# menyifang/MIMO

Hardware: NVIDIA H100
Metric: frames/sec @ 512x512x24f, 20 DDIM steps (higher is better)
Workload: dtype fp16

## Files before the change

### include/mimo_b200.h

```cpp
#ifndef MIMO_B200_H_
#define MIMO_B200_H_

#include <stdint.h>

#ifdef __cplusplus
extern "C" {
#endif

#define MIMO_OK 0
#define MIMO_ERR_ARG (-1)
#define MIMO_ERR_CUDA (-2)
#define MIMO_ERR_DEVICE (-3)

#define MIMO_F16 0
#define MIMO_BF16 1

#define MIMO_ACT_NONE 0
#define MIMO_ACT_SILU 1
#define MIMO_ACT_GEGLU 2

const char* mimo_version(void);
const char* mimo_last_error(void);
int mimo_device_check(int dev);
int mimo_abi_sizeof(int which);

typedef struct {
  const void* bias;
  const void* rowvec;
  int64_t rows_per_group;
  int64_t ld_rowvec;
  const void* residual;
  int64_t ld_res;
  float scale;
  int act;
} mimo_epilogue;

typedef struct {
  const void* a;
  int64_t lda;
  const void* a1;
  int64_t lda1;
  const void* w;
  int64_t ldw;
  void* out;
  int64_t ldo;
  int32_t M, N, K;
  int32_t K1;
  int32_t dtype;
  mimo_epilogue ep;
  void* workspace;
  int64_t workspace_bytes;
} mimo_gemm_params;
int mimo_gemm(const mimo_gemm_params* p, void* stream);
int mimo_gemm_geglu_granule(int32_t N);

typedef struct {
  const void* a;
  int64_t lda;
  const float* a_scale;
  const void* w;
  int64_t ldw;
  const float* w_scale;
  void* out;
  int64_t ldo;
  int32_t M, N, K;
  int32_t dtype;
  mimo_epilogue ep;
  void* workspace;
  int64_t workspace_bytes;
} mimo_gemm_e4m3_params;
int mimo_gemm_e4m3(const mimo_gemm_e4m3_params* p, void* stream);

typedef struct {
  const void* x0;
  int32_t c0;
  const void* x1;
  int32_t c1;
  const void* w;
  void* out;
  int64_t ldo;
  int32_t n, h, w_, cout;
  int32_t dtype;
  mimo_epilogue ep;
  void* workspace;
  int64_t workspace_bytes;
} mimo_conv3x3_params;
int mimo_conv3x3(const mimo_conv3x3_params* p, void* stream);
// ... 155 lines not shown
```

### mimo_b200/csrc/gemm_wgmma.cu

```cuda
#include <cuda_runtime.h>

#include <cudaTypedefs.h>

#include "../../include/mimo_b200.h"
#include "host_util.h"
#include "ptx.cuh"
#include "wgmma.cuh"

namespace mimo {

constexpr int BM = 128;
constexpr int BK = 64;
constexpr int kGemmThreads = 320;
constexpr int kChunk = 8192;

struct EpiArgs {
  const void* bias;
  const void* rowvec;
  long long rows_per_group;
  long long ld_rowvec;
  float scale;
  int act;
  float* partial;
};
// ... 23 lines not shown
  static constexpr int kResBytes = kResSlots * kChunk;
  static constexpr int kBarBytes = 512;
  static constexpr int kFixed = kBarBytes + 2048  + (kE4m3 ? 3072  : 0) + kOutBytes + kResBytes;
  static constexpr int kMaxStages = (BN >= 256) ? 4 : (BN >= 160 ? 5 : (BN >= 128 ? 6 : 8));
  static constexpr int kFit = (227 * 1024 - kFixed) / kStageBytes;
  static constexpr int kStages = kFit < kMaxStages ? kFit : kMaxStages;
  static constexpr int kSmemBytes = kStages * kStageBytes + kFixed;
  static_assert(kStages >= 3, "pipeline too shallow");
};

template <int BN, bool kBf16, bool kRes>
__global__ void __launch_bounds__(kGemmThreads, 1)
gemm_wgmma_kernel(const __grid_constant__ CUtensorMap tmA0, const __grid_constant__ CUtensorMap tmA1,
                  const __grid_constant__ CUtensorMap tmB, const __grid_constant__ CUtensorMap tmOut,
                  const __grid_constant__ CUtensorMap tmRes, int M, int N, int num_m_tiles, int num_n_tiles,
                  int num_k_blocks, ConvGeom g, EpiArgs ep) {
  constexpr bool kE4m3 = false;
  constexpr const float* a_scale = nullptr;
  constexpr const float* w_scale = nullptr;
#include "gemm_wgmma_body.cuh"
}

template <int BN, bool kBf16, bool kRes>
__global__ void __launch_bounds__(kGemmThreads, 1)
gemm_e4m3_kernel(const __grid_constant__ CUtensorMap tmA0, const __grid_constant__ CUtensorMap tmA1,
                 const __grid_constant__ CUtensorMap tmB, const __grid_constant__ CUtensorMap tmOut,
                 const __grid_constant__ CUtensorMap tmRes, int M, int N, int num_m_tiles, int num_n_tiles,
                 int num_k_blocks, ConvGeom g, EpiArgs ep, const float* __restrict__ a_scale,
                 const float* __restrict__ w_scale) {
  constexpr bool kE4m3 = true;
#include "gemm_wgmma_body.cuh"
}


template <bool kBf16>
__global__ void __launch_bounds__(256)
splitk_reduce_kernel(const float* __restrict__ part, int splits, long long M, int N, const void* __restrict__ bias,
                     const void* __restrict__ rowvec, long long rpg, long long ld_rowvec,
                     const void* __restrict__ res, long long ld_res, float scale, int act, void* __restrict__ out,
                     long long ldo) {
  using C = Cvt<kBf16>;
  using T = typename C::T;
  pdl_launch_dependents();
  pdl_wait();
  const int nv = N >> 3;
  const long long idx = blockIdx.x * static_cast<long long>(blockDim.x) + threadIdx.x;
  if (idx >= M * nv) return;
  const long long row = idx / nv;
  const int col = static_cast<int>(idx - row * nv) * 8;
  float a[8] = {0.f, 0.f, 0.f, 0.f, 0.f, 0.f, 0.f, 0.f};
  for (int s = 0; s < splits; ++s) {
    const float4* p = reinterpret_cast<const float4*>(part + (static_cast<long long>(s) * M + row) * N + col);
    const float4 u0 = p[0], u1 = p[1];
    a[0] += u0.x, a[1] += u0.y, a[2] += u0.z, a[3] += u0.w;
    a[4] += u1.x, a[5] += u1.y, a[6] += u1.z, a[7] += u1.w;
  }
  float cst[8] = {0.f, 0.f, 0.f, 0.f, 0.f, 0.f, 0.f, 0.f};
  auto add_vec = [&](const T* v, float* dst, bool scaled_fma) {
    const uint4 b = *reinterpret_cast<const uint4*>(v);
    const uint32_t w[4] = {b.x, b.y, b.z, b.w};
#pragma unroll
    for (int j = 0; j < 4; ++j) {
      const float2 t = C::unpack(w[j]);
      if (scaled_fma) {
        dst[2 * j] = fmaf(t.x, scale, dst[2 * j]);
        dst[2 * j + 1] = fmaf(t.y, scale, dst[2 * j + 1]);
// ... 47 lines not shown
  }
  const int tiles = mt * nt;
  const int grid = tiles < num_sms() ? tiles : num_sms();
  cudaError_t e = launch_k(kern, dim3(grid), dim3(kGemmThreads), Cfg::kSmemBytes, st, m.a0, m.a1, m.b, m.out, m.res, M, N, mt,
                           nt, nkb, g, ep);
  if (e == cudaSuccess) e = cudaGetLastError();
  if (e != cudaSuccess) return set_cuda_error("gemm launch", e);
  return MIMO_OK;
}

template <bool kBf16>
static int launch_bn(int bn, bool res, const Maps& m, int M, int N, int mt, int nt, int nkb, const ConvGeom& g,
                     const EpiArgs& ep, cudaStream_t st) {
  switch (bn) {
    case 64:
      return res ? launch_cfg<64, kBf16, true>(m, M, N, mt, nt, nkb, g, ep, st)
                 : launch_cfg<64, kBf16, false>(m, M, N, mt, nt, nkb, g, ep, st);
    case 128:
      return res ? launch_cfg<128, kBf16, true>(m, M, N, mt, nt, nkb, g, ep, st)
                 : launch_cfg<128, kBf16, false>(m, M, N, mt, nt, nkb, g, ep, st);
    case 160:
      return res ? launch_cfg<160, kBf16, true>(m, M, N, mt, nt, nkb, g, ep, st)
                 : launch_cfg<160, kBf16, false>(m, M, N, mt, nt, nkb, g, ep, st);
    case 192:
      return res ? launch_cfg<192, kBf16, true>(m, M, N, mt, nt, nkb, g, ep, st)
                 : launch_cfg<192, kBf16, false>(m, M, N, mt, nt, nkb, g, ep, st);
    case 256:
      return res ? launch_cfg<256, kBf16, true>(m, M, N, mt, nt, nkb, g, ep, st)
                 : launch_cfg<256, kBf16, false>(m, M, N, mt, nt, nkb, g, ep, st);
  }
  return set_error(MIMO_ERR_ARG, "gemm: unsupported BN");
}

int pick_bn(int N, bool geglu, long long m_tiles);

template <bool kBf16>
static int launch_e4m3(int bn, bool res, const Maps& m, int M, int N, int mt, int nt, int nkb, const ConvGeom& g,
                       const EpiArgs& ep, const float* a_scale, const float* w_scale, cudaStream_t st) {
  auto run = [&](auto kern, int smem) -> int {
    static bool attr_done[2][2][2] = {};
    bool& done = attr_done[bn == 256][kBf16][res];
    if (!done) {
      cudaError_t e = cudaFuncSetAttribute(kern, cudaFuncAttributeMaxDynamicSharedMemorySize, smem);
      if (e != cudaSuccess) return set_cuda_error("cudaFuncSetAttribute(gemm_e4m3)", e);
      done = true;
    }
    const int tiles = mt * nt;
    const int grid = tiles < num_sms() ? tiles : num_sms();
    cudaError_t e = launch_k(kern, dim3(grid), dim3(kGemmThreads), smem, st, m.a0, m.a1, m.b, m.out, m.res, M, N, mt, nt,
                             nkb, g, ep, a_scale, w_scale);
    if (e == cudaSuccess) e = cudaGetLastError();
    if (e != cudaSuccess) return set_cuda_error("gemm_e4m3 launch", e);
    return MIMO_OK;
  };
  if (bn == 192)
    return res ? run(gemm_e4m3_kernel<192, kBf16, true>, GemmCfg<192, true, true>::kSmemBytes)
               : run(gemm_e4m3_kernel<192, kBf16, false>, GemmCfg<192, false, true>::kSmemBytes);
  if (bn == 256)
    return res ? run(gemm_e4m3_kernel<256, kBf16, true>, GemmCfg<256, true, true>::kSmemBytes)
               : run(gemm_e4m3_kernel<256, kBf16, false>, GemmCfg<256, false, true>::kSmemBytes);
  return set_error(MIMO_ERR_ARG, "mimo_gemm_e4m3: unsupported BN");
}

static int pick_bn_e4m3(int N, bool geglu) {
  if (geglu) return pick_bn(N, true, 1 << 20);
  const int pad256 = (N + 255) / 256 * 256 - N, pad192 = (N + 191) / 192 * 192 - N;
  return pad192 < pad256 ? 192 : 256;
}

static int g_force_bn = 0;

int pick_bn(int N, bool geglu, long long m_tiles) {
  if (g_force_bn) return g_force_bn;
  if (geglu) {
    if (N % 256 == 0) return 256;
    if (N % 128 == 0) return 128;
    return 64;
  }
  const int cands[5] = {256, 192, 160, 128, 64};
  int best = 64;
  double best_eff = -1.0;
  for (int i = 0; i < 5; ++i) {
    const int bn = cands[i];
    const int nt = (N + bn - 1) / bn;
    double eff = static_cast<double>(N) / (static_cast<double>(nt) * bn);
    const long long tiles = m_tiles * nt;
    if (tiles < num_sms() && bn > 64) eff *= 0.5 + 0.5 * static_cast<double>(tiles) / num_sms();
    if (eff > best_eff + 1e-9) {
      best_eff = eff;
      best = bn;
    }
  }
  return best;
}

static EpiArgs make_epi(const mimo_epilogue& e, int N) {
  EpiArgs a;
  a.bias = e.bias;
  a.rowvec = e.rowvec;
  a.rows_per_group = e.rows_per_group > 0 ? e.rows_per_group : 1;
  if (a.rows_per_group > 0x7fffffffLL) a.rows_per_group = 0x7fffffffLL;
  a.ld_rowvec = e.ld_rowvec > 0 ? e.ld_rowvec : N;
  a.scale = e.scale;
  a.act = e.act;
  a.partial = nullptr;
  return a;
}

static int g_splitk = 0;

static int launch_reduce(int dtype, const float* part, int splits, long long M, int N, const mimo_epilogue& e, void* out,
                         long long ldo, cudaStream_t st) {
  const long long total = M * (N / 8);
  const unsigned blocks = div_up(total, 256);
  const long long rpg = e.rows_per_group > 0 ? e.rows_per_group : 1;
  const long long ldr = e.ld_rowvec > 0 ? e.ld_rowvec : N;
  cudaError_t err = dtype == MIMO_BF16
                        ? launch_k(splitk_reduce_kernel<true>, dim3(blocks), dim3(256), 0, st, part, splits, M, N, e.bias,
                                   e.rowvec, rpg, ldr, e.residual, static_cast<long long>(e.ld_res), e.scale, e.act, out, ldo)
                        : launch_k(splitk_reduce_kernel<false>, dim3(blocks), dim3(256), 0, st, part, splits, M, N, e.bias,
                                   e.rowvec, rpg, ldr, e.residual, static_cast<long long>(e.ld_res), e.scale, e.act, out, ldo);
  if (err == cudaSuccess) err = cudaGetLastError();
  if (err != cudaSuccess) return set_cuda_error("split-K reduce launch", err);
  return MIMO_OK;
}

}

using namespace mimo;

extern "C" int mimo_debug_splitk(int mode) {
  g_splitk = mode;
  return 0;
}

extern "C" int mimo_debug_force_bn(int bn) {
  g_force_bn = bn;
  return 0;
}

extern "C" int mimo_gemm_geglu_granule(int32_t N) { return pick_bn(N, true, 1 << 20) / 2; }

extern "C" int mimo_gemm(const mimo_gemm_params* p, void* stream) {
  if (!p || !p->a || !p->w || !p->out) return set_error(MIMO_ERR_ARG, "mimo_gemm: null pointer");
  if (p->M <= 0 || p->N <= 0 || p->K <= 0) return set_error(MIMO_ERR_ARG, "mimo_gemm: empty problem");
  if ((p->K % 8) || (p->lda % 8) || (p->ldw % 8) || (p->N % 8) || (p->ldo % 8))
    return set_error(MIMO_ERR_ARG, "mimo_gemm: K, N, lda, ldw, ldo must be multiples of 8");
  if (p->ep.residual && (p->ep.ld_res % 8)) return set_error(MIMO_ERR_ARG, "mimo_gemm: ld_res % 8 != 0");
  const bool geglu = p->ep.act == MIMO_ACT_GEGLU;
  if (geglu && (p->ep.residual || p->ep.rowvec))
    return set_error(MIMO_ERR_ARG, "mimo_gemm: GEGLU takes neither a residual nor a row vector");
  if (int rc = ensure_device()) return rc;
  const int mt = (p->M + BM - 1) / BM;
  const int K1 = p->a1 ? p->K1 : 0;
  if (K1 < 0 || (K1 % 8) || (p->a1 && (p->lda1 % 8))) return set_error(MIMO_ERR_ARG, "mimo_gemm: K1/lda1 % 8 != 0");
  const int kb0 = (p->K + BK - 1) / BK;
  const int kb1 = (K1 + BK - 1) / BK;
  const int nkb = kb0 + kb1;
  int bn = pick_bn(p->N, geglu, mt);
  int splits = 1;
  if (!geglu && g_splitk && p->workspace && !g_force_bn) {
    const int bn_wide = pick_bn(p->N, false, 1 << 20);
    splits = pick_splits(static_cast<long long>(mt) * ((p->N + bn_wide - 1) / bn_wide), nkb, p->M, p->N, p->workspace_bytes);
    if (splits > 1) bn = bn_wide;
  }
  if (geglu && (p->N % bn)) return set_error(MIMO_ERR_ARG, "mimo_gemm: GEGLU needs N % tile == 0");
  const int nt = (p->N + bn - 1) / bn;
  const bool res = p->ep.residual != nullptr && !geglu && splits == 1;

  Maps m;
  const uint64_t adim[2] = {static_cast<uint64_t>(p->K), static_cast<uint64_t>(p->M)};
  const uint64_t astr[1] = {static_cast<uint64_t>(p->lda) * 2};
  const uint32_t abox[2] = {BK, BM};
  if (int rc = encode_tmap(&m.a0, p->dtype, 2, p->a, adim, astr, abox)) return rc;
  m.a1 = m.a0;
  if (K1) {
    const uint64_t a1dim[2] = {static_cast<uint64_t>(K1), static_cast<uint64_t>(p->M)};
    const uint64_t a1str[1] = {static_cast<uint64_t>(p->lda1) * 2};
    if (int rc = encode_tmap(&m.a1, p->dtype, 2, p->a1, a1dim, a1str, abox)) return rc;
  }
  const uint64_t bdim[2] = {static_cast<uint64_t>(p->K + K1), static_cast<uint64_t>(p->N)};
  const uint64_t bstr[1] = {static_cast<uint64_t>(p->ldw) * 2};
  const uint32_t bbox[2] = {BK, static_cast<uint32_t>(bn)};
  if (int rc = encode_tmap(&m.b, p->dtype, 2, p->w, bdim, bstr, bbox)) return rc;
  const int n_out = geglu ? p->N / 2 : p->N;
  const uint64_t odim[2] = {static_cast<uint64_t>(n_out), static_cast<uint64_t>(p->M)};
  const uint64_t ostr[1] = {static_cast<uint64_t>(p->ldo) * 2};
  const uint32_t obox[2] = {32, BM};
  if (int rc = encode_tmap(&m.out, p->dtype, 2, p->out, odim, ostr, obox, 64)) return rc;
  m.res = m.out;
  if (res) {
    const uint64_t rstr[1] = {static_cast<uint64_t>(p->ep.ld_res) * 2};
    if (int rc = encode_tmap(&m.res, p->dtype, 2, p->ep.residual, odim, rstr, obox, 64)) return rc;
  }

  ConvGeom g = {};
  g.kb0 = kb0;
  g.kb1 = kb1;
  g.c0 = p->K;
  g.chunk_bytes = kChunk;
  g.splits = splits;
  g.kb_split = (nkb + splits - 1) / splits;
  EpiArgs ep = make_epi(p->ep, p->N);
  cudaStream_t st = static_cast<cudaStream_t>(stream);
  if (splits > 1) {
    ep.bias = ep.rowvec = nullptr;
    ep.act = MIMO_ACT_NONE;
    ep.scale = 1.0f;
    ep.partial = static_cast<float*>(p->workspace);
  }
  const int rc = p->dtype == MIMO_BF16 ? launch_bn<true>(bn, res, m, p->M, p->N, mt, nt, nkb, g, ep, st)
                                       : launch_bn<false>(bn, res, m, p->M, p->N, mt, nt, nkb, g, ep, st);
  if (rc || splits == 1) return rc;
  return launch_reduce(p->dtype, ep.partial, splits, p->M, p->N, p->ep, p->out, p->ldo, st);
}

extern "C" int mimo_gemm_e4m3(const mimo_gemm_e4m3_params* p, void* stream) {
  if (!p || !p->a || !p->w || !p->out || !p->a_scale || !p->w_scale)
    return set_error(MIMO_ERR_ARG, "mimo_gemm_e4m3: null pointer");
  if (p->M <= 0 || p->N <= 0 || p->K <= 0) return set_error(MIMO_ERR_ARG, "mimo_gemm_e4m3: empty problem");
  if ((p->K % 16) || (p->lda % 16) || (p->ldw % 16))
    return set_error(MIMO_ERR_ARG, "mimo_gemm_e4m3: K, lda, ldw must be multiples of 16");
  if ((p->N % 8) || (p->ldo % 8)) return set_error(MIMO_ERR_ARG, "mimo_gemm_e4m3: N, ldo must be multiples of 8");
  if ((reinterpret_cast<uintptr_t>(p->a) | reinterpret_cast<uintptr_t>(p->w) | reinterpret_cast<uintptr_t>(p->out) |
       reinterpret_cast<uintptr_t>(p->ep.residual)) % 16)
    return set_error(MIMO_ERR_ARG, "mimo_gemm_e4m3: a, w, out, residual must be 16-byte aligned");
  if (p->ep.residual && (p->ep.ld_res % 8)) return set_error(MIMO_ERR_ARG, "mimo_gemm_e4m3: ld_res % 8 != 0");
  if (p->workspace || p->workspace_bytes) return set_error(MIMO_ERR_ARG, "mimo_gemm_e4m3: split-K is not supported");
  const bool geglu = p->ep.act == MIMO_ACT_GEGLU;
  if (geglu && (p->ep.residual || p->ep.rowvec))
    return set_error(MIMO_ERR_ARG, "mimo_gemm_e4m3: GEGLU takes neither a residual nor a row vector");
  const int bn = pick_bn_e4m3(p->N, geglu);
  if (geglu && (p->N % bn)) return set_error(MIMO_ERR_ARG, "mimo_gemm_e4m3: GEGLU needs N % tile == 0");
  if (bn != 192 && bn != 256) return set_error(MIMO_ERR_ARG, "mimo_gemm_e4m3: GEGLU needs N % 256 == 0");
  if (int rc = ensure_device()) return rc;
  const int mt = (p->M + BM - 1) / BM;
  const int nt = (p->N + bn - 1) / bn;
  const int nkb = (p->K + 2 * BK - 1) / (2 * BK);
  const bool res = p->ep.residual != nullptr && !geglu;

  Maps m;
  const uint64_t adim[2] = {static_cast<uint64_t>(p->K), static_cast<uint64_t>(p->M)};
  const uint64_t astr[1] = {static_cast<uint64_t>(p->lda)};
// ... 40 lines not shown
  if (g.TH < 1) g.TH = 1;
  g.TN = BM / (g.TW * g.TH);
  if (g.TN > p->n) g.TN = p->n;
  if (g.TN < 1) g.TN = 1;
  if (g.TN > 1 && g.TH != p->h) g.TN = 1;
  g.tiles_w = (p->w_ + g.TW - 1) / g.TW;
  g.tiles_h = (p->h + g.TH - 1) / g.TH;
  const int tiles_n = (p->n + g.TN - 1) / g.TN;
  g.ctot = p->c0 + c1;
  g.c0 = p->c0;
  g.kb0 = (p->c0 + BK - 1) / BK;
  g.kb1 = (c1 + BK - 1) / BK;
  g.a_bytes = g.TW * g.TH * g.TN * BK * 2;
  g.chunk_bytes = g.TW * g.TH * g.TN * 64;
  g.ntaps = ntaps;
  for (int t = 0; t < 9; ++t) {
    g.tdx[t] = t < ntaps ? tdx[t] : 0;
    g.tdy[t] = t < ntaps ? tdy[t] : 0;
  }
  const int mt = g.tiles_w * g.tiles_h * tiles_n;
  const int nkb = ntaps * (g.kb0 + g.kb1);
  const long long Mrows = static_cast<long long>(p->n) * p->h * p->w_;
  if (Mrows > 0x7fffffffLL) return set_error(MIMO_ERR_ARG, "mimo_conv: too many pixels");
  int bn = pick_bn(p->cout, false, mt);
  int splits = 1;
  if (g_splitk && p->workspace && !g_force_bn && sx == 1 && sy == 1 && p->ldo == p->cout) {
    const int bn_wide = pick_bn(p->cout, false, 1 << 20);
    splits = pick_splits(static_cast<long long>(mt) * ((p->cout + bn_wide - 1) / bn_wide), nkb, Mrows, p->cout,
                         p->workspace_bytes);
    if (splits > 1) bn = bn_wide;
  }
  g.splits = splits;
  g.kb_split = (nkb + splits - 1) / splits;
  const int nt = (p->cout + bn - 1) / bn;
  const bool res = p->ep.residual != nullptr && splits == 1;

  Maps m;
  auto nhwc_map = [&](CUtensorMap* tm, const void* base, int c, long long pitch, uint32_t box_c, int swz, int px,
                      int py, int iw, int ih) {
    const uint64_t dim[4] = {static_cast<uint64_t>(c), static_cast<uint64_t>(p->w_), static_cast<uint64_t>(p->h),
                             static_cast<uint64_t>(p->n)};
    const uint64_t str[3] = {static_cast<uint64_t>(px) * pitch * 2, static_cast<uint64_t>(py) * iw * pitch * 2,
                             static_cast<uint64_t>(ih) * iw * pitch * 2};
    const uint32_t box[4] = {box_c, static_cast<uint32_t>(g.TW), static_cast<uint32_t>(g.TH),
                             static_cast<uint32_t>(g.TN)};
    return encode_tmap(tm, p->dtype, 4, base, dim, str, box, swz);
  };
  if (int rc = nhwc_map(&m.a0, p->x0, p->c0, p->c0, BK, 128, 1, 1, p->w_, p->h)) return rc;
  m.a1 = m.a0;
  if (c1)
    if (int rc = nhwc_map(&m.a1, p->x1, c1, c1, BK, 128, 1, 1, p->w_, p->h)) return rc;
  {
    const uint64_t dim[2] = {static_cast<uint64_t>(ntaps) * g.ctot, static_cast<uint64_t>(p->cout)};
    const uint64_t str[1] = {static_cast<uint64_t>(ntaps) * g.ctot * 2};
    const uint32_t box[2] = {BK, static_cast<uint32_t>(bn)};
    if (int rc = encode_tmap(&m.b, p->dtype, 2, w, dim, str, box)) return rc;
  }
  if (int rc = nhwc_map(&m.out, out, p->cout, p->ldo, 32, 64, sx, sy, ow, oh)) return rc;
  m.res = m.out;
  if (res)
    if (int rc = nhwc_map(&m.res, p->ep.residual, p->cout, p->ep.ld_res, 32, 64, 1, 1, p->w_, p->h)) return rc;

  EpiArgs ep = make_epi(p->ep, p->cout);
  cudaStream_t st = static_cast<cudaStream_t>(stream);
  if (splits > 1) {
    ep.bias = ep.rowvec = nullptr;
    ep.act = MIMO_ACT_NONE;
    ep.scale = 1.0f;
    ep.partial = static_cast<float*>(p->workspace);
  }
  const int rc = p->dtype == MIMO_BF16
                     ? launch_bn<true>(bn, res, m, static_cast<int>(Mrows), p->cout, mt, nt, nkb, g, ep, st)
                     : launch_bn<false>(bn, res, m, static_cast<int>(Mrows), p->cout, mt, nt, nkb, g, ep, st);
  if (rc || splits == 1) return rc;
  return launch_reduce(p->dtype, ep.partial, splits, Mrows, p->cout, p->ep, out, p->ldo, st);
}

static int conv_check(const mimo_conv3x3_params* p, const char* who) {
  if (!p || !p->x0 || !p->w || !p->out) return set_error(MIMO_ERR_ARG, "mimo_conv: null pointer");
  if (p->n <= 0 || p->h <= 0 || p->w_ <= 0 || p->cout <= 0 || p->c0 <= 0)
    return set_error(MIMO_ERR_ARG, "mimo_conv: empty problem");
  const int c1 = p->x1 ? p->c1 : 0;
  if ((p->c0 % 8) || (c1 % 8) || (p->cout % 8) || (p->ldo % 8))
    return set_error(MIMO_ERR_ARG, "mimo_conv: channel counts must be multiples of 8");
  if (p->ep.act == MIMO_ACT_GEGLU) return set_error(MIMO_ERR_ARG, "mimo_conv: GEGLU not supported");
  if (p->ep.residual && (p->ep.ld_res % 8)) return set_error(MIMO_ERR_ARG, "mimo_conv: ld_res % 8 != 0");
  (void)who;
  return ensure_device();
}

extern "C" int mimo_conv3x3(const mimo_conv3x3_params* p, void* stream) {
  if (int rc = conv_check(p, "mimo_conv3x3")) return rc;
  static const signed char dx[9] = {-1, 0, 1, -1, 0, 1, -1, 0, 1};
  static const signed char dy[9] = {-1, -1, -1, 0, 0, 0, 1, 1, 1};
  return conv_launch(p, p->w, 9, dx, dy, p->out, 1, 1, p->w_, p->h, stream);
}

extern "C" int mimo_conv_up2x(const mimo_conv3x3_params* p, void* stream) {
  if (int rc = conv_check(p, "mimo_conv_up2x")) return rc;
  if (p->ep.residual || p->ep.rowvec) return set_error(MIMO_ERR_ARG, "mimo_conv_up2x: bias / activation epilogue only");
  const int ctot = p->c0 + (p->x1 ? p->c1 : 0);
  const size_t esz = 2;
  for (int a = 0; a < 2; ++a)
// ... 12 lines not shown
```

### mimo_b200/csrc/ptx.cuh

```cuda
#pragma once
#include <cuda_fp16.h>
#include <cuda_bf16.h>
#include <cuda.h>
#include <stdint.h>
#include <stdio.h>

namespace mimo {

__device__ __forceinline__ uint32_t smem_u32(const void* p) {
  return static_cast<uint32_t>(__cvta_generic_to_shared(p));
}
__device__ __forceinline__ uint32_t lane_id() { return threadIdx.x & 31u; }

__device__ __forceinline__ bool elect_one() {
  uint32_t pred = 0;
  asm volatile(
      "{\n\t.reg .pred P;\n\telect.sync _|P, 0xffffffff;\n\tselp.u32 %0, 1, 0, P;\n\t}\n"
      : "=r"(pred));
  return pred != 0;
}

__device__ __forceinline__ void pdl_launch_dependents() { asm volatile("griddepcontrol.launch_dependents;" ::: "memory"); }
__device__ __forceinline__ void pdl_wait() { asm volatile("griddepcontrol.wait;" ::: "memory"); }

// ... 10 lines not shown
}
__device__ __forceinline__ void mbar_arrive(uint64_t* bar) {
  asm volatile("mbarrier.arrive.shared::cta.b64 _, [%0];" ::"r"(smem_u32(bar)) : "memory");
}
__device__ __forceinline__ bool mbar_try_wait(uint64_t* bar, uint32_t parity) {
  uint32_t ok;
  asm volatile(
      "{\n\t.reg .pred p;\n\t"
      "mbarrier.try_wait.parity.shared::cta.b64 p, [%1], %2;\n\t"
      "selp.u32 %0, 1, 0, p;\n\t}\n"
      : "=r"(ok)
      : "r"(smem_u32(bar)), "r"(parity)
      : "memory");
  return ok != 0;
}
__device__ __forceinline__ bool mbar_test(uint64_t* bar, uint32_t parity) {
  uint32_t ok;
  asm volatile(
      "{\n\t.reg .pred p;\n\t"
      "mbarrier.test_wait.parity.shared::cta.b64 p, [%1], %2;\n\t"
      "selp.u32 %0, 1, 0, p;\n\t}\n"
      : "=r"(ok)
      : "r"(smem_u32(bar)), "r"(parity)
      : "memory");
  return ok != 0;
}
__device__ __forceinline__ void mbar_wait(uint64_t* bar, uint32_t parity) {
  uint32_t spins = 0;
  while (!mbar_try_wait(bar, parity)) {
    if (++spins > (1u << 26)) __trap();
  }
}

__device__ __forceinline__ void fence_proxy_async_smem() {
  asm volatile("fence.proxy.async.shared::cta;" ::: "memory");
}

__device__ __forceinline__ void tma_prefetch_desc(const CUtensorMap* m) {
  asm volatile("prefetch.tensormap [%0];" ::"l"(reinterpret_cast<uint64_t>(m)) : "memory");
}
__device__ __forceinline__ void tma_load_2d(void* smem_dst, const CUtensorMap* m, uint64_t* bar,
                                            int32_t c0, int32_t c1) {
  asm volatile(
      "cp.async.bulk.tensor.2d.shared::cluster.global.mbarrier::complete_tx::bytes"
      " [%0], [%1, {%3, %4}], [%2];"
      ::"r"(smem_u32(smem_dst)), "l"(reinterpret_cast<uint64_t>(m)), "r"(smem_u32(bar)), "r"(c0),
      "r"(c1)
      : "memory");
}
__device__ __forceinline__ void tma_load_3d(void* smem_dst, const CUtensorMap* m, uint64_t* bar,
                                            int32_t c0, int32_t c1, int32_t c2) {
  asm volatile(
      "cp.async.bulk.tensor.3d.shared::cluster.global.mbarrier::complete_tx::bytes"
      " [%0], [%1, {%3, %4, %5}], [%2];"
      ::"r"(smem_u32(smem_dst)), "l"(reinterpret_cast<uint64_t>(m)), "r"(smem_u32(bar)), "r"(c0),
      "r"(c1), "r"(c2)
      : "memory");
}
__device__ __forceinline__ void tma_load_4d(void* smem_dst, const CUtensorMap* m, uint64_t* bar,
                                            int32_t c0, int32_t c1, int32_t c2, int32_t c3) {
  asm volatile(
      "cp.async.bulk.tensor.4d.shared::cluster.global.mbarrier::complete_tx::bytes"
      " [%0], [%1, {%3, %4, %5, %6}], [%2];"
      ::"r"(smem_u32(smem_dst)), "l"(reinterpret_cast<uint64_t>(m)), "r"(smem_u32(bar)), "r"(c0),
      "r"(c1), "r"(c2), "r"(c3)
      : "memory");
}

__device__ __forceinline__ void tma_store_2d(const CUtensorMap* m, const void* smem_src, int32_t c0, int32_t c1) {
  asm volatile("cp.async.bulk.tensor.2d.global.shared::cta.bulk_group [%0, {%2, %3}], [%1];"
               ::"l"(reinterpret_cast<uint64_t>(m)), "r"(smem_u32(smem_src)), "r"(c0), "r"(c1)
               : "memory");
}
__device__ __forceinline__ void tma_store_4d(const CUtensorMap* m, const void* smem_src, int32_t c0, int32_t c1,
                                             int32_t c2, int32_t c3) {
  asm volatile("cp.async.bulk.tensor.4d.global.shared::cta.bulk_group [%0, {%2, %3, %4, %5}], [%1];"
               ::"l"(reinterpret_cast<uint64_t>(m)), "r"(smem_u32(smem_src)), "r"(c0), "r"(c1), "r"(c2), "r"(c3)
               : "memory");
}
__device__ __forceinline__ void tma_store_commit() { asm volatile("cp.async.bulk.commit_group;" ::: "memory"); }
__device__ __forceinline__ void tma_store_wait_read0() { asm volatile("cp.async.bulk.wait_group.read 0;" ::: "memory"); }
__device__ __forceinline__ void tma_store_wait_all() { asm volatile("cp.async.bulk.wait_group 0;" ::: "memory"); }

__device__ __forceinline__ void wgmma_fence() { asm volatile("wgmma.fence.sync.aligned;" ::: "memory"); }
__device__ __forceinline__ void wgmma_commit() { asm volatile("wgmma.commit_group.sync.aligned;" ::: "memory"); }
template <int N>
__device__ __forceinline__ void wgmma_wait() {
  asm volatile("wgmma.wait_group.sync.aligned %0;" ::"n"(N) : "memory");
}
template <int N>
__device__ __forceinline__ void reg_fence(float (&d)[N]) {
#pragma unroll
  for (int i = 0; i < N; ++i) asm volatile("" : "+f"(d[i])::"memory");
}

__device__ __forceinline__ void bar_sync(int id, int count) {
  asm volatile("bar.sync %0, %1;" ::"r"(id), "r"(count) : "memory");
}
__device__ __forceinline__ void bar_arrive(int id, int count) {
  asm volatile("bar.arrive %0, %1;" ::"r"(id), "r"(count) : "memory");
}

__device__ __forceinline__ uint64_t make_smem_desc_sw128(uint32_t smem_addr, uint32_t lbo_bytes,
                                                         uint32_t sbo_bytes) {
  uint64_t d = 0;
  d |= static_cast<uint64_t>((smem_addr & 0x3FFFFu) >> 4);
  d |= static_cast<uint64_t>((lbo_bytes >> 4) & 0x3FFFu) << 16;
  d |= static_cast<uint64_t>((sbo_bytes >> 4) & 0x3FFFu) << 32;
  d |= static_cast<uint64_t>(1) << 62;
  return d;
}

__device__ __forceinline__ float ex2_ftz(float x) {
  float y;
  asm("ex2.approx.ftz.f32 %0, %1;" : "=f"(y) : "f"(x));
  return y;
}
__device__ __forceinline__ float silu_f(float x) { return __fdividef(x, 1.0f + __expf(-x)); }
__device__ __forceinline__ float gelu_erf_f(float x) {
  return 0.5f * x * (1.0f + erff(x * 0.70710678118654752440f));
}

__device__ __forceinline__ float gelu_erf_fast(float x) {
  const float z = fabsf(x) * 0.70710678118654752440f;
  float t;
  asm("rcp.approx.ftz.f32 %0, %1;" : "=f"(t) : "f"(fmaf(0.3275911f, z, 1.0f)));
  float poly = fmaf(1.061405429f, t, -1.453152027f);
// ... 44 lines not shown
```

### mimo_b200/lib.py

```python
from __future__ import annotations

import ctypes as C
import os
from pathlib import Path

_PKG = Path(__file__).resolve().parent
LIB_PATH = _PKG / "libmimo_b200.so"

F16, BF16 = 0, 1
ACT_NONE, ACT_SILU, ACT_GEGLU = 0, 1, 2


class MimoError(RuntimeError):
    pass


class Epilogue(C.Structure):
    _fields_ = [
        ("bias", C.c_void_p),
        ("rowvec", C.c_void_p),
        ("rows_per_group", C.c_int64),
        ("ld_rowvec", C.c_int64),
        ("residual", C.c_void_p),
        ("ld_res", C.c_int64),
# ... 98 lines not shown

MAX_PEERS = 8


class ExchangeParams(C.Structure):
    _fields_ = [
        ("peer_src", C.c_void_p * MAX_PEERS), ("peer_ready", C.c_void_p * MAX_PEERS),
        ("ctl", C.c_void_p), ("dst", C.c_void_p), ("residual", C.c_void_p),
        ("mode", C.c_int32), ("G", C.c_int32), ("r", C.c_int32),
        ("b", C.c_int32), ("fl", C.c_int32), ("hw", C.c_int32), ("C", C.c_int32),
        ("dtype", C.c_int32), ("max_blocks", C.c_int32), ("timeout_ms", C.c_int32),
    ]


class CfgMultistepParams(C.Structure):
    _fields_ = [
        ("pred_uncond", C.c_void_p), ("pred_cond", C.c_void_p), ("counter", C.c_void_p), ("frame_stride", C.c_int64),
        ("latents", C.c_void_p), ("count", C.c_int64),
        ("hist_out", C.c_void_p), ("h1", C.c_void_p), ("h2", C.c_void_p), ("noise", C.c_void_p),
        ("guidance", C.c_float), ("a", C.c_float), ("b", C.c_float),
        ("c_x", C.c_float), ("c_m", C.c_float), ("c_1", C.c_float), ("c_2", C.c_float), ("c_n", C.c_float),
        ("dtype", C.c_int32),
    ]


_VP, _I32, _I64, _F = C.c_void_p, C.c_int32, C.c_int64, C.c_float
SYMBOLS = {
    "mimo_version": (C.c_char_p, []),
    "mimo_last_error": (C.c_char_p, []),
    "mimo_device_check": (C.c_int, [C.c_int]),
    "mimo_abi_sizeof": (C.c_int, [C.c_int]),
    "mimo_gemm": (C.c_int, [C.POINTER(GemmParams), _VP]),
    "mimo_gemm_geglu_granule": (C.c_int, [_I32]),
    "mimo_gemm_e4m3": (C.c_int, [C.POINTER(GemmE4m3Params), _VP]),
    "mimo_conv3x3": (C.c_int, [C.POINTER(Conv3x3Params), _VP]),
    "mimo_conv_up2x": (C.c_int, [C.POINTER(Conv3x3Params), _VP]),
    "mimo_im2col3x3": (C.c_int, [_VP, _VP, _I32, _I32, _I32, _I32, _I32, _I32, _I32, _I64, _I32, _VP]),
    "mimo_groupnorm": (C.c_int, [C.POINTER(GroupNormParams), _VP]),
    "mimo_groupnorm_workspace_bytes": (C.c_int64, [C.POINTER(GroupNormParams)]),
    "mimo_groupnorm_window": (C.c_int, [C.POINTER(GroupNormWindowParams), _VP]),
    "mimo_groupnorm_window_partials": (C.c_int, [C.POINTER(GroupNormWindowParams), _VP]),
    "mimo_groupnorm_window_apply": (C.c_int, [C.POINTER(GroupNormWindowParams), _VP]),
    "mimo_groupnorm_window_table_bytes": (C.c_int64, [C.POINTER(GroupNormWindowParams)]),
    "mimo_layernorm": (C.c_int, [_VP, _VP, _VP, _VP, _I64, _I32, _F, _VP, _I64, _I32, _I32, _I32, _VP]),
    "mimo_layernorm_e4m3": (C.c_int, [_VP, _VP, _VP, _VP, _VP, _I64, _I32, _F, _VP, _I64, _I32, _I32, _I32, _VP]),
    "mimo_attn_spatial": (C.c_int, [C.POINTER(AttnParams), _VP]),
    "mimo_attn_temporal": (C.c_int, [C.POINTER(AttnTemporalParams), _VP]),
    "mimo_exchange": (C.c_int, [C.POINTER(ExchangeParams), _VP]),
    "mimo_peer_alloc": (C.c_int, [_I64, C.POINTER(C.c_void_p), C.c_char_p]),
    "mimo_peer_open": (C.c_int, [C.c_char_p, C.POINTER(C.c_void_p)]),
    "mimo_peer_close": (C.c_int, [_VP]),
    "mimo_peer_free": (C.c_int, [_VP]),
    "mimo_ncfhw_to_nhwc": (C.c_int, [_VP, _VP, _I32, _I32, _I32, _I32, _I32, _I32, _I32, _I32, _VP]),
    "mimo_nhwc_to_ncfhw": (C.c_int, [_VP, _VP, _I32, _I32, _I32, _I32, _I32, _I32, _I32, _I32, _VP]),
    "mimo_upsample2x": (C.c_int, [_VP, _VP, _I32, _I32, _I32, _I32, _I32, _VP]),
    "mimo_upsample_nearest": (C.c_int, [_VP, _VP, _I32, _I32, _I32, _I32, _I32, _I32, _I32, _VP]),
    "mimo_softmax_rows": (C.c_int, [_VP, _I64, _I32, _I64, _I32, _VP]),
    "mimo_add": (C.c_int, [_VP, _VP, _VP, _I64, _I32, _VP]),
    "mimo_silu": (C.c_int, [_VP, _VP, _I64, _I32, _VP]),
    "mimo_quick_gelu": (C.c_int, [_VP, _VP, _I64, _I32, _VP]),
    "mimo_composite_frame": (C.c_int, [_VP, _VP, _VP, _VP, _VP, _VP, C.c_double, _VP, _I64, _VP]),
    "mimo_cfg_ddim_step": (C.c_int, [_VP, _VP, _VP, _I64, _VP, _I64, _F, _F, _F, _F, _F, _I32, _VP]),
    "mimo_cfg_ddim_step_noise": (C.c_int, [_VP, _VP, _VP, _I64, _VP, _I64, _F, _F, _F, _F, _F, _VP, _F, _I32, _VP]),
    "mimo_interpolate_frames": (C.c_int, [_VP, _VP, _I32, _I64, _I32, _I32, _I32, _VP]),
    "mimo_cfg_multistep": (C.c_int, [C.POINTER(CfgMultistepParams), _VP]),
}
# ... 36 lines not shown
```

Measured before the change: 8.198.

## Add persistent warp-specialized ping-pong WGMMA GEMM/conv kernel with wider N tiles

Adds a persistent ping-pong kernel. A producer warp issues TMA loads and another warp prefetches the residual. Two consumer warpgroups alternate tiles, so one warpgroup's epilogue overlaps the other's main loop, and registers are rebalanced with setmaxnreg. A heuristic routes non-split GEMMs and 3x3 convs to it with BN of 128, 160 or 192, plus a GEGLU granule path. The goal is to hide epilogue and store latency and to raise tensor-core utilisation, at the cost of more complex synchronisation and shallower pipelines for wide tiles.

```diff
diff --git a/include/mimo_b200.h b/include/mimo_b200.h
--- a/include/mimo_b200.h
+++ b/include/mimo_b200.h
@@ -53,6 +53,7 @@
 } mimo_gemm_params;
 int mimo_gemm(const mimo_gemm_params* p, void* stream);
 int mimo_gemm_geglu_granule(int32_t N);
+int mimo_debug_gemm_schedule(int mode);
 
 typedef struct {
   const void* a;
diff --git a/mimo_b200/csrc/gemm_wgmma.cu b/mimo_b200/csrc/gemm_wgmma.cu
--- a/mimo_b200/csrc/gemm_wgmma.cu
+++ b/mimo_b200/csrc/gemm_wgmma.cu
@@ -79,6 +79,390 @@
 #include "gemm_wgmma_body.cuh"
 }
 
+
+constexpr int kPingPongThreads = 384;
+
+template <int BN, bool kRes>
+struct PingPongCfg {
+  static constexpr int kStageBytes = BM * BK * 2 + BN * BK * 2;
+  static constexpr int kNChunk = BN / 32;
+  static constexpr int kOutBytes = 2 * 2 * kChunk;
+  static constexpr int kResSlots = kRes ? 2 : 0;
+  static constexpr int kResBytes = 2 * kResSlots * kChunk;
+  static constexpr int kBarBytes = 512;
+  static constexpr int kFixed = kBarBytes + 2048  + kOutBytes + kResBytes;
+  static constexpr int kMaxStages = BN >= 160 ? 5 : (BN >= 128 ? 6 : 8);
+  static constexpr int kFit = (227 * 1024 - kFixed) / kStageBytes;
+  static constexpr int kStages = kFit < kMaxStages ? kFit : kMaxStages;
+  static constexpr int kSmemBytes = kStages * kStageBytes + kFixed;
+  static_assert(kStages >= 3, "pipeline too shallow");
+  static_assert(BN <= 192, "BN accumulators per thread must fit the 232-register consumers");
+};
+
+template <int BN, bool kBf16, bool kRes>
+__global__ void __launch_bounds__(kPingPongThreads, 1)
+gemm_pingpong_kernel(const __grid_constant__ CUtensorMap tmA0, const __grid_constant__ CUtensorMap tmA1,
+                     const __grid_constant__ CUtensorMap tmB, const __grid_constant__ CUtensorMap tmOut,
+                     const __grid_constant__ CUtensorMap tmRes, int M, int N, int num_m_tiles, int num_n_tiles,
+                     int num_k_blocks, ConvGeom g, EpiArgs ep, int w_granule) {
+  using Cfg = PingPongCfg<BN, kRes>;
+  using C = Cvt<kBf16>;
+  using T = typename C::T;
+  constexpr int NCHUNK = Cfg::kNChunk;
+  extern __shared__ __align__(1024) uint8_t smem[];
+  uint8_t* sOut = smem + Cfg::kStages * Cfg::kStageBytes;
+  uint8_t* sRes = sOut + Cfg::kOutBytes;
+  uint64_t* bars = reinterpret_cast<uint64_t*>(sRes + Cfg::kResBytes);
+  uint64_t* full_bar = bars;
+  uint64_t* empty_bar = bars + 8;
+  uint64_t* res_full = bars + 16;
+  uint64_t* res_empty = bars + 20;
+  float* sbias = reinterpret_cast<float*>(reinterpret_cast<uint8_t*>(bars) + Cfg::kBarBytes);
+
+  pdl_launch_dependents();
+  const int warp = __shfl_sync(0xffffffffu, threadIdx.x >> 5, 0);
+  const int lane = threadIdx.x & 31;
+  const int num_tiles = num_m_tiles * num_n_tiles;
+  const bool geglu = ep.act == MIMO_ACT_GEGLU;
+
+  if (warp == 8 && lane == 0) {
+    tma_prefetch_desc(&tmA0);
+    tma_prefetch_desc(&tmA1);
+    tma_prefetch_desc(&tmB);
+    tma_prefetch_desc(&tmOut);
+    if (kRes) tma_prefetch_desc(&tmRes);
+  }
+  if (warp == 9 && lane == 0) {
+    for (int s = 0; s < Cfg::kStages; ++s) {
+      mbar_init(&full_bar[s], 1);
+      mbar_init(&empty_bar[s], 4);
+    }
+    for (int s = 0; s < 2 * Cfg::kResSlots; ++s) {
+      mbar_init(&res_full[s], 1);
+      mbar_init(&res_empty[s], 4);
+    }
+    fence_mbar_init();
+  }
+  __syncthreads();
+  pdl_wait();
+
+  auto tile_origin = [&](int m_tile, int& x0, int& y0, int& n0) {
+    if (g.conv) {
+      x0 = (m_tile % g.tiles_w) * g.TW;
+      y0 = ((m_tile / g.tiles_w) % g.tiles_h) * g.TH;
+      n0 = (m_tile / (g.tiles_w * g.tiles_h)) * g.TN;
+    } else {
+      x0 = y0 = n0 = 0;
+    }
+  };
+  auto w_row0 = [&](int n_tile) {
+    return w_granule ? (n_tile * 64 / w_granule) * 2 * w_granule + (n_tile * 64) % w_granule : n_tile * BN;
+  };
+
+  if (warp >= 8) {
+    setmaxnreg_dec<40>();
+    if (warp == 8) {
+      uint32_t stage = 0, phase = 0;
+      const int kb_per_tap = g.kb0 + g.kb1;
+      for (int tile = blockIdx.x; tile < num_tiles; tile += gridDim.x) {
+        const int m_tile = tile / num_n_tiles, n_tile = tile - m_tile * num_n_tiles;
+        int x0, y0, n0;
+        tile_origin(m_tile, x0, y0, n0);
+        const int wn0 = w_row0(n_tile);
+        int tap = 0, rem = 0, dx = g.tdx[0], dy = g.tdy[0], tap_k = 0;
+        for (int kb = 0; kb < num_k_blocks; ++kb) {
+          mbar_wait(&empty_bar[stage], phase ^ 1u);
+          uint8_t* sa = smem + stage * Cfg::kStageBytes;
+          uint8_t* sb = sa + BM * BK * 2;
+          if (elect_one()) {
+            auto load_w = [&](int kcoord) {
+              tma_load_2d(sb, &tmB, &full_bar[stage], kcoord, wn0);
+              if (w_granule) tma_load_2d(sb + 64 * BK * 2, &tmB, &full_bar[stage], kcoord, wn0 + w_granule);
+            };
+            if (!g.conv) {
+              mbar_expect_tx(&full_bar[stage], BM * BK * 2 + BN * BK * 2);
+              if (kb < g.kb0) {
+                tma_load_2d(sa, &tmA0, &full_bar[stage], kb * BK, m_tile * BM);
+                load_w(kb * BK);
+              } else {
+                tma_load_2d(sa, &tmA1, &full_bar[stage], (kb - g.kb0) * BK, m_tile * BM);
+                load_w(g.c0 + (kb - g.kb0) * BK);
+              }
+            } else {
+              mbar_expect_tx(&full_bar[stage], g.a_bytes + BN * BK * 2);
+              if (rem < g.kb0) {
+                tma_load_4d(sa, &tmA0, &full_bar[stage], rem * BK, x0 + dx, y0 + dy, n0);
+                load_w(tap_k + rem * BK);
+              } else {
+                tma_load_4d(sa, &tmA1, &full_bar[stage], (rem - g.kb0) * BK, x0 + dx, y0 + dy, n0);
+                load_w(tap_k + g.c0 + (rem - g.kb0) * BK);
+              }
+            }
+          }
+          __syncwarp();
+          if (++rem == kb_per_tap) {
+            rem = 0;
+            tap_k += g.ctot;
+            if (++tap == g.ntaps) tap = 0;
+            dx = g.tdx[tap];
+            dy = g.tdy[tap];
+          }
+          if (++stage == Cfg::kStages) {
+            stage = 0;
+            phase ^= 1u;
+          }
+        }
+      }
+      for (int s = 0; s < Cfg::kStages; ++s) {
+        mbar_wait(&empty_bar[stage], phase ^ 1u);
+        if (++stage == Cfg::kStages) {
+          stage = 0;
+          phase ^= 1u;
+        }
+      }
+    } else if (warp == 9) {
+      if constexpr (kRes) {
+        int lt = 0;
+        for (int tile = blockIdx.x; tile < num_tiles; tile += gridDim.x, ++lt) {
+          const int m_tile = tile / num_n_tiles, n_tile = tile - m_tile * num_n_tiles;
+          int x0, y0, n0;
+          tile_origin(m_tile, x0, y0, n0);
+          const int w = lt & 1;
+          for (int c = 0; c < NCHUNK; ++c) {
+            const uint32_t k = static_cast<uint32_t>(lt >> 1) * NCHUNK + c;
+            const uint32_t slot = w * Cfg::kResSlots + k % Cfg::kResSlots;
+            mbar_wait(&res_empty[slot], ((k / Cfg::kResSlots) & 1u) ^ 1u);
+            if (elect_one()) {
+              mbar_expect_tx(&res_full[slot], g.chunk_bytes);
+              const int col = n_tile * BN + c * 32;
+              if (g.conv)
+                tma_load_4d(sRes + slot * kChunk, &tmRes, &res_full[slot], col, x0, y0, n0);
+              else
+                tma_load_2d(sRes + slot * kChunk, &tmRes, &res_full[slot], col, m_tile * BM);
+            }
+            __syncwarp();
+          }
+        }
+        for (int w = 0; w < 2; ++w) {
+          const uint32_t k_end = static_cast<uint32_t>((lt + 1 - w) / 2) * NCHUNK;
+          for (uint32_t k = k_end; k < k_end + Cfg::kResSlots; ++k)
+            mbar_wait(&res_empty[w * Cfg::kResSlots + k % Cfg::kResSlots], ((k / Cfg::kResSlots) & 1u) ^ 1u);
+        }
+      }
+    }
+    return;
+  }
+
+  setmaxnreg_inc<232>();
+  const int wg = warp >> 2;
+  const int ct = threadIdx.x & 127;
+  const int bar_main = 1 + wg, bar_main_other = 2 - wg, bar_wg = 3 + wg;
+  const int rbase = (warp & 3) * 16 + (lane >> 2);
+  const int q2 = (lane & 3) * 2;
+  const bool issuer = ct == 0;
+  const int sw[2] = {(rbase >> 1) & 3, ((rbase + 8) >> 1) & 3};
+  const bool do_silu = ep.act == MIMO_ACT_SILU;
+  const uint32_t rpg = static_cast<uint32_t>(ep.rows_per_group);
+  uint8_t* const wout = sOut + wg * 2 * kChunk;
+  uint8_t* const wres = sRes + wg * Cfg::kResSlots * kChunk;
+  uint64_t* const wres_full = res_full + wg * Cfg::kResSlots;
+  uint64_t* const wres_empty = res_empty + wg * Cfg::kResSlots;
+  float* const sb = sbias + wg * 256;
+  float acc[2][BN / 2];
+  uint32_t stage = (wg * num_k_blocks) % Cfg::kStages, phase = ((wg * num_k_blocks) / Cfg::kStages) & 1u;
+  uint32_t oc = 0, rc = 0;
+
+  for (int tile = blockIdx.x + wg * gridDim.x, lt = wg; tile < num_tiles; tile += 2 * gridDim.x, lt += 2) {
+    const int m_tile = tile / num_n_tiles, n_tile = tile - m_tile * num_n_tiles;
+    const bool partner_next = tile + static_cast<int>(gridDim.x) < num_tiles;
+    int x0, y0, n0;
+    tile_origin(m_tile, x0, y0, n0);
+    auto tile_groups = [&](int mt, uint32_t& gf, uint32_t& gl) {
+      if (!g.conv) {
+        const uint32_t m0 = static_cast<uint32_t>(mt) * BM;
+        uint32_t m1 = m0 + BM - 1;
+        if (m1 > static_cast<uint32_t>(M) - 1) m1 = static_cast<uint32_t>(M) - 1;
+        gf = m0 / rpg;
+        gl = m1 / rpg;
+      } else {
+        int tx, ty, tn;
+        tile_origin(mt, tx, ty, tn);
+        int n1 = tn + g.TN - 1;
+        if (n1 > g.NI - 1) n1 = g.NI - 1;
+        const uint32_t hw = static_cast<uint32_t>(g.H) * g.W;
+        gf = (static_cast<uint32_t>(tn) * hw) / rpg;
+        gl = (static_cast<uint32_t>(n1 + 1) * hw - 1) / rpg;
+      }
+    };
+    {
+      const int wn0 = w_row0(n_tile);
+      for (int c = ct; c < BN; c += 128) {
+        const int col = w_granule ? wn0 + (c < 64 ? c : w_granule + c - 64) : wn0 + c;
+        float v = 0.f;
+        if (col < N) {
+          if (ep.bias) v = C::to_f(static_cast<const T*>(ep.bias)[col]);
+          if (ep.rowvec) {
+            uint32_t gf, gl;
+            tile_groups(m_tile, gf, gl);
+            if (gf == gl) v += C::to_f(static_cast<const T*>(ep.rowvec)[static_cast<long long>(gf) * ep.ld_rowvec + col]);
+          }
+        }
+        sb[c] = geglu ? v : v * ep.scale;
+      }
+    }
+
+    if (lt > 0) bar_sync(bar_main, 256);
+    uint32_t prev_stage = 0;
+    for (int kb = 0; kb < num_k_blocks; ++kb) {
+      mbar_wait_spin(&full_bar[stage], phase);
+      const uint32_t sa = smem_u32(smem + stage * Cfg::kStageBytes);
+      const uint64_t da0 = make_smem_desc_sw128(sa, 16, 1024);
+      const uint64_t da1 = make_smem_desc_sw128(sa + 64 * 128, 16, 1024);
+      const uint64_t db = make_smem_desc_sw128(sa + BM * BK * 2, 16, 1024);
+      wgmma_fence();
+#pragma unroll
+      for (int k = 0; k < BK / 16; ++k) {
+        Wgmma<BN, kBf16>::ss(acc[0], da0 + 2 * k, db + 2 * k, (kb | k) != 0 ? 1u : 0u);
+        Wgmma<BN, kBf16>::ss(acc[1], da1 + 2 * k, db + 2 * k, (kb | k) != 0 ? 1u : 0u);
+      }
+      wgmma_commit();
+      if (kb > 0) {
+        wgmma_wait<1>();
+        if (lane == 0) mbar_arrive(&empty_bar[prev_stage]);
+      }
+      prev_stage = stage;
+      if (++stage == Cfg::kStages) {
+        stage = 0;
+        phase ^= 1u;
+      }
+    }
+    if (partner_next) bar_arrive(bar_main_other, 256);
+    wgmma_wait<0>();
+    reg_fence(acc[0]);
+    reg_fence(acc[1]);
+    if (lane == 0) mbar_arrive(&empty_bar[prev_stage]);
+    stage += num_k_blocks;
+    phase ^= (stage / Cfg::kStages) & 1u;
+    stage %= Cfg::kStages;
+
+    bar_sync(bar_wg, 128);
+
+    auto stage_and_store = [&](uint8_t* obuf, int col0) {
+      fence_proxy_async_smem();
+      if (issuer) tma_store_wait_read0();
+      bar_sync(bar_wg, 128);
+      if (issuer) {
+        if (g.conv)
+          tma_store_4d(&tmOut, obuf, col0, x0, y0, n0);
+        else
+          tma_store_2d(&tmOut, obuf, col0, m_tile * BM);
+        tma_store_commit();
+      }
+    };
+
+    if (!geglu) {
+      const float scale = ep.scale;
+      bool rv_uniform = false;
+      if (ep.rowvec) {
+        uint32_t gf, gl;
+        tile_groups(m_tile, gf, gl);
+        rv_uniform = gf == gl;
+      }
+      const bool need_rv = ep.rowvec != nullptr && !rv_uniform;
+      const int mode = (!kRes && !do_silu && !need_rv && ep.bias == nullptr && ep.rowvec == nullptr && scale == 1.0f)
+                           ? 0 : (need_rv ? 2 : 1);
+      const T* rv[4];
+#pragma unroll
+      for (int i = 0; i < 4; ++i) {
+        const int r = 64 * (i >> 1) + rbase + 8 * (i & 1);
+        long long row;
+        bool row_ok;
+        if (!g.conv) {
+          row = static_cast<long long>(m_tile) * BM + r;
+          row_ok = row < M;
+        } else {
+          const int x = r % g.TW, y = (r / g.TW) % g.TH, n = r / (g.TW * g.TH);
+          row_ok = (n < g.TN) && (x0 + x < g.W) && (y0 + y < g.H) && (n0 + n < g.NI);
+          row = (static_cast<long long>(n0 + n) * g.H + (y0 + y)) * g.W + (x0 + x);
+        }
+        rv[i] = (need_rv && row_ok)
+                    ? static_cast<const T*>(ep.rowvec) + static_cast<long long>(static_cast<uint32_t>(row) / rpg) * ep.ld_rowvec
+                    : nullptr;
+      }
+#pragma unroll
+      for (int c = 0; c < NCHUNK; ++c) {
+        uint8_t* obuf = wout + (oc & 1u) * kChunk;
+        ++oc;
+        const int col0 = n_tile * BN + c * 32;
+        [[maybe_unused]] uint32_t rslot = 0;
+        if constexpr (kRes) {
+          const uint32_t k = rc++;
+          rslot = k % Cfg::kResSlots;
+          mbar_wait_spin(&wres_full[rslot], (k / Cfg::kResSlots) & 1u);
+        }
+#pragma unroll
+        for (int jj = 0; jj < 4; ++jj) {
+          const int j = 4 * c + jj;
+          const float2 cst0 = *reinterpret_cast<const float2*>(sb + c * 32 + 8 * jj + q2);
+#pragma unroll
+          for (int i = 0; i < 4; ++i) {
+            const int h2 = i >> 1, h = i & 1;
+            const int r = 64 * h2 + rbase + 8 * h;
+            const int off = r * 64 + ((jj ^ sw[h]) << 4) + q2 * 2;
+            float f0 = acc[h2][4 * j + 2 * h], f1 = acc[h2][4 * j + 2 * h + 1];
+            if (mode != 0) {
+              float c0 = cst0.x, c1 = cst0.y;
+              if (mode == 2 && rv[i] && col0 + 8 * jj + q2 < N) {
+                const float2 t = C::unpack(__ldg(reinterpret_cast<const unsigned int*>(rv[i] + col0 + 8 * jj + q2)));
+                c0 = fmaf(t.x, scale, c0);
+                c1 = fmaf(t.y, scale, c1);
+              }
+              f0 = fmaf(f0, scale, c0);
+              f1 = fmaf(f1, scale, c1);
+            }
+            if constexpr (kRes) {
+              const float2 t = C::unpack(*reinterpret_cast<const uint32_t*>(wres + rslot * kChunk + off));
+              f0 = fmaf(t.x, scale, f0);
+              f1 = fmaf(t.y, scale, f1);
+            }
+            if (do_silu) {
+              f0 = silu_f(f0);
+              f1 = silu_f(f1);
+            }
+            *reinterpret_cast<uint32_t*>(obuf + off) = C::pack(f0, f1);
+          }
+        }
+        if constexpr (kRes) {
+          __syncwarp();
+          if (lane == 0) mbar_arrive(&wres_empty[rslot]);
+        }
+        stage_and_store(obuf, col0);
+      }
+    } else if constexpr (BN == 128) {
+#pragma unroll
+      for (int c = 0; c < 2; ++c) {
+        uint8_t* obuf = wout + (oc & 1u) * kChunk;
+        ++oc;
+#pragma unroll
+        for (int jj = 0; jj < 4; ++jj) {
+          const int j = 4 * c + jj, jg = j + 8;
+          const float2 cv = *reinterpret_cast<const float2*>(sb + c * 32 + 8 * jj + q2);
+          const float2 cg = *reinterpret_cast<const float2*>(sb + 64 + c * 32 + 8 * jj + q2);
+#pragma unroll
+          for (int i = 0; i < 4; ++i) {
+            const int h2 = i >> 1, h = i & 1;
+            const int r = 64 * h2 + rbase + 8 * h;
+            const float f0 = (acc[h2][4 * j + 2 * h] + cv.x) * gelu_erf_fast(acc[h2][4 * jg + 2 * h] + cg.x);
+            const float f1 = (acc[h2][4 * j + 2 * h + 1] + cv.y) * gelu_erf_fast(acc[h2][4 * jg + 2 * h + 1] + cg.y);
+            *reinterpret_cast<uint32_t*>(obuf + r * 64 + ((jj ^ sw[h]) << 4) + q2 * 2) = C::pack(f0, f1);
+          }
+        }
+        stage_and_store(obuf, n_tile * 64 + c * 32);
+      }
+    }
+  }
+  if (issuer) tma_store_wait_all();
+}
 
 template <bool kBf16>
 __global__ void __launch_bounds__(256)
@@ -192,6 +576,42 @@
   return set_error(MIMO_ERR_ARG, "gemm: unsupported BN");
 }
 
+template <int BN, bool kBf16, bool kRes>
+static int launch_pp_cfg(const Maps& m, int M, int N, int mt, int nt, int nkb, const ConvGeom& g, const EpiArgs& ep,
+                         int w_granule, cudaStream_t st) {
+  using Cfg = PingPongCfg<BN, kRes>;
+  auto kern = gemm_pingpong_kernel<BN, kBf16, kRes>;
+  static bool attr_done = false;
+  if (!attr_done) {
+    cudaError_t e = cudaFuncSetAttribute(kern, cudaFuncAttributeMaxDynamicSharedMemorySize, Cfg::kSmemBytes);
+    if (e != cudaSuccess) return set_cuda_error("cudaFuncSetAttribute(gemm_pingpong)", e);
+    attr_done = true;
+  }
+  const int tiles = mt * nt;
+  const int grid = tiles < num_sms() ? tiles : num_sms();
+  cudaError_t e = launch_k(kern, dim3(grid), dim3(kPingPongThreads), Cfg::kSmemBytes, st, m.a0, m.a1, m.b, m.out, m.res, M,
+                           N, mt, nt, nkb, g, ep, w_granule);
+  if (e == cudaSuccess) e = cudaGetLastError();
+  if (e != cudaSuccess) return set_cuda_error("gemm_pingpong launch", e);
+  return MIMO_OK;
+}
+
+template <bool kBf16>
+static int launch_pp(int bn, bool res, const Maps& m, int M, int N, int mt, int nt, int nkb, const ConvGeom& g,
+                     const EpiArgs& ep, int w_granule, cudaStream_t st) {
+  switch (bn) {
+    case 128:
+      return res ? launch_pp_cfg<128, kBf16, true>(m, M, N, mt, nt, nkb, g, ep, w_granule, st)
+                 : launch_pp_cfg<128, kBf16, false>(m, M, N, mt, nt, nkb, g, ep, w_granule, st);
+    case 160:
+      return res ? launch_pp_cfg<160, kBf16, true>(m, M, N, mt, nt, nkb, g, ep, w_granule, st)
+                 : launch_pp_cfg<160, kBf16, false>(m, M, N, mt, nt, nkb, g, ep, w_granule, st);
+    case 192:
+      if (!res) return launch_pp_cfg<192, kBf16, false>(m, M, N, mt, nt, nkb, g, ep, w_granule, st);
+  }
+  return set_error(MIMO_ERR_ARG, "gemm: unsupported ping-pong BN");
+}
+
 int pick_bn(int N, bool geglu, long long m_tiles);
 
 template <bool kBf16>
@@ -254,6 +674,30 @@
   return best;
 }
 
+static int g_gemm_schedule = 1;
+
+static int pick_bn_pingpong(int N, int geglu_granule, bool res, long long m_tiles, int nkb) {
+  if (!g_gemm_schedule) return 0;
+  if (!g_force_bn && (geglu_granule ? nkb >= 20 : nkb <= 5)) return 0;
+  if (geglu_granule) return geglu_granule % 64 == 0 ? 128 : 0;
+  if (g_force_bn) return (g_force_bn == 128 || g_force_bn == 160 || (g_force_bn == 192 && !res)) ? g_force_bn : 0;
+  if (pick_bn(N, false, m_tiles) == 64) return 0;
+  const int cands[3] = {192, 160, 128};
+  int best = 0;
+  double best_eff = -1.0;
+  for (int bn : cands) {
+    const int nt = (N + bn - 1) / bn;
+    double eff = static_cast<double>(N) / (static_cast<double>(nt) * bn);
+    const long long tiles = m_tiles * nt;
+    if (tiles < num_sms()) eff *= 0.5 + 0.5 * static_cast<double>(tiles) / num_sms();
+    if (eff > best_eff + 1e-9) {
+      best_eff = eff;
+      best = bn;
+    }
+  }
+  return res && best == 192 ? 0 : best;
+}
+
 static EpiArgs make_epi(const mimo_epilogue& e, int N) {
   EpiArgs a;
   a.bias = e.bias;
@@ -296,6 +740,12 @@
 
 extern "C" int mimo_debug_force_bn(int bn) {
   g_force_bn = bn;
+  return 0;
+}
+
+extern "C" int mimo_debug_gemm_schedule(int mode) {
+  if (mode != 0 && mode != 1) return set_error(MIMO_ERR_ARG, "mimo_debug_gemm_schedule: mode must be 0 or 1");
+  g_gemm_schedule = mode;
   return 0;
 }
 
@@ -325,6 +775,9 @@
     if (splits > 1) bn = bn_wide;
   }
   if (geglu && (p->N % bn)) return set_error(MIMO_ERR_ARG, "mimo_gemm: GEGLU needs N % tile == 0");
+  const int pp_bn = splits == 1 ? pick_bn_pingpong(p->N, geglu ? bn / 2 : 0, p->ep.residual != nullptr && !geglu, mt, nkb) : 0;
+  const int w_granule = pp_bn && geglu ? bn / 2 : 0;
+  if (pp_bn) bn = pp_bn;
   const int nt = (p->N + bn - 1) / bn;
   const bool res = p->ep.residual != nullptr && !geglu && splits == 1;
 
@@ -341,7 +794,7 @@
   }
   const uint64_t bdim[2] = {static_cast<uint64_t>(p->K + K1), static_cast<uint64_t>(p->N)};
   const uint64_t bstr[1] = {static_cast<uint64_t>(p->ldw) * 2};
-  const uint32_t bbox[2] = {BK, static_cast<uint32_t>(bn)};
+  const uint32_t bbox[2] = {BK, static_cast<uint32_t>(w_granule ? 64 : bn)};
   if (int rc = encode_tmap(&m.b, p->dtype, 2, p->w, bdim, bstr, bbox)) return rc;
   const int n_out = geglu ? p->N / 2 : p->N;
   const uint64_t odim[2] = {static_cast<uint64_t>(n_out), static_cast<uint64_t>(p->M)};
@@ -369,6 +822,9 @@
     ep.scale = 1.0f;
     ep.partial = static_cast<float*>(p->workspace);
   }
+  if (pp_bn)
+    return p->dtype == MIMO_BF16 ? launch_pp<true>(bn, res, m, p->M, p->N, mt, nt, nkb, g, ep, w_granule, st)
+                                 : launch_pp<false>(bn, res, m, p->M, p->N, mt, nt, nkb, g, ep, w_granule, st);
   const int rc = p->dtype == MIMO_BF16 ? launch_bn<true>(bn, res, m, p->M, p->N, mt, nt, nkb, g, ep, st)
                                        : launch_bn<false>(bn, res, m, p->M, p->N, mt, nt, nkb, g, ep, st);
   if (rc || splits == 1) return rc;
@@ -475,6 +931,8 @@
   }
   g.splits = splits;
   g.kb_split = (nkb + splits - 1) / splits;
+  const int pp_bn = splits == 1 ? pick_bn_pingpong(p->cout, 0, p->ep.residual != nullptr, mt, nkb) : 0;
+  if (pp_bn) bn = pp_bn;
   const int nt = (p->cout + bn - 1) / bn;
   const bool res = p->ep.residual != nullptr && splits == 1;
 
@@ -512,6 +970,10 @@
     ep.scale = 1.0f;
     ep.partial = static_cast<float*>(p->workspace);
   }
+  if (pp_bn)
+    return p->dtype == MIMO_BF16
+               ? launch_pp<true>(bn, res, m, static_cast<int>(Mrows), p->cout, mt, nt, nkb, g, ep, 0, st)
+               : launch_pp<false>(bn, res, m, static_cast<int>(Mrows), p->cout, mt, nt, nkb, g, ep, 0, st);
   const int rc = p->dtype == MIMO_BF16
                      ? launch_bn<true>(bn, res, m, static_cast<int>(Mrows), p->cout, mt, nt, nkb, g, ep, st)
                      : launch_bn<false>(bn, res, m, static_cast<int>(Mrows), p->cout, mt, nt, nkb, g, ep, st);
diff --git a/mimo_b200/csrc/ptx.cuh b/mimo_b200/csrc/ptx.cuh
--- a/mimo_b200/csrc/ptx.cuh
+++ b/mimo_b200/csrc/ptx.cuh
@@ -66,6 +66,11 @@
   }
 }
 
+__device__ __forceinline__ void mbar_wait_spin(uint64_t* bar, uint32_t parity) {
+  while (!mbar_try_wait(bar, parity)) {
+  }
+}
+
 __device__ __forceinline__ void fence_proxy_async_smem() {
   asm volatile("fence.proxy.async.shared::cta;" ::: "memory");
 }
@@ -127,6 +132,11 @@
 #pragma unroll
   for (int i = 0; i < N; ++i) asm volatile("" : "+f"(d[i])::"memory");
 }
+
+template <uint32_t N>
+__device__ __forceinline__ void setmaxnreg_inc() { asm volatile("setmaxnreg.inc.sync.aligned.u32 %0;" ::"n"(N)); }
+template <uint32_t N>
+__device__ __forceinline__ void setmaxnreg_dec() { asm volatile("setmaxnreg.dec.sync.aligned.u32 %0;" ::"n"(N)); }
 
 __device__ __forceinline__ void bar_sync(int id, int count) {
   asm volatile("bar.sync %0, %1;" ::"r"(id), "r"(count) : "memory");
diff --git a/mimo_b200/lib.py b/mimo_b200/lib.py
--- a/mimo_b200/lib.py
+++ b/mimo_b200/lib.py
@@ -154,6 +154,7 @@
     "mimo_abi_sizeof": (C.c_int, [C.c_int]),
     "mimo_gemm": (C.c_int, [C.POINTER(GemmParams), _VP]),
     "mimo_gemm_geglu_granule": (C.c_int, [_I32]),
+    "mimo_debug_gemm_schedule": (C.c_int, [C.c_int]),
     "mimo_gemm_e4m3": (C.c_int, [C.POINTER(GemmE4m3Params), _VP]),
     "mimo_conv3x3": (C.c_int, [C.POINTER(Conv3x3Params), _VP]),
     "mimo_conv_up2x": (C.c_int, [C.POINTER(Conv3x3Params), _VP]),
```

New measurement: 8.419 (median of 6 runs). 1.03x the previous value.
